# sovrasov/3d-object-detection.pytorch

Hardware: AMD Instinct MI355X
Metric: regression train crops/sec @224^2 bs256 MobileNetV2 (higher is better)
Workload: dtype bf16; 1 GPU; mobilenetv2 9-class Objectron keypoint regression, train step (fwd + l1/add/CE losses + bwd + AdamW), 224x224 crops, per-GPU batch 256; global_batch=256, parallelism=dp1, roofline_sampled_steps=0, rccl_ranks=0

## Files before the change

### 3d-object-detection.pytorch_amd/csrc/bn.hip

```cpp
#include "common.h"

namespace {

__device__ __forceinline__ void load_sums(const double* __restrict__ stats, int nrep, long long rstride, int C, int c, int rl,
                                          double& s1, double& s2) {
  s1 = 0.0;
  s2 = 0.0;
  if (c < C) {
    for (int r = rl; r < nrep; r += 16) {
      s1 += stats[r * rstride + c];
      s2 += stats[r * rstride + C + c];
    }
  }
#pragma unroll
  for (int o = 8; o > 0; o >>= 1) {
    s1 += __shfl_xor(s1, o, 16);
    s2 += __shfl_xor(s2, o, 16);
  }
}

__global__ void bn_finalize_kernel(const double* __restrict__ stats, int nrep, long long rstride, int C, double count,
                                   const float* __restrict__ gamma, const float* __restrict__ beta,
                                   float* running_mean, float* running_var, int64_t* nbt, float momentum,
                                   float eps, float* scale, float* shift, float* mean_out, float* invstd_out) {
// ... 50 lines not shown
__global__ void bn_bwd_finalize_kernel(const double* __restrict__ stats, int nrep, long long rstride, int C, double count,
                                       const float* __restrict__ gamma, const float* __restrict__ mean,
                                       const float* __restrict__ invstd, float* alpha, float* beta, float* gammac,
                                       float* dgamma, float* dbeta) {
  const int c = blockIdx.x * 16 + (threadIdx.x >> 4), rl = threadIdx.x & 15;
  double s1, s2;
  load_sums(stats, nrep, rstride, C, c, rl, s1, s2);
  if (c >= C || rl != 0) return;
  const double mu = (double)mean[c], is = (double)invstd[c];
  const double dg = is * (s2 - mu * s1);
  const double a = (double)(gamma ? gamma[c] : 1.f) * is;
  const double b = -a * is * dg / count;
  alpha[c] = (float)a;
  beta[c] = (float)b;
  gammac[c] = (float)(-a * s1 / count - b * mu);
  if (dgamma) dgamma[c] = (float)dg;
  if (dbeta) dbeta[c] = (float)s1;
}

__global__ __launch_bounds__(256) void bn_fold_kernel(const T3dFold* __restrict__ fp) {
  __shared__ float sink[3 * 64];
  const int C = fp->C, cbase = blockIdx.x * 64;
  if (cbase >= C) return;
  t3d_fold_block(fp, cbase, min(64, C - cbase), sink, 64, true);
}

}

int t3d_fold_fallback(const void* key, hipStream_t st) {
  const T3dFold* d = t3d_take_fold(key);
  if (!d) return T3D_OK;
  T3D_LAUNCH(bn_fold_kernel, dim3(32), dim3(256), 0, st, d);
  T3D_CHECK_LAUNCH();
  return T3D_OK;
}

extern "C" int t3d_bn_finalize(const double* stats, int C, double count, const float* gamma, const float* beta,
                               float* running_mean, float* running_var, int64_t* num_batches_tracked,
                               float momentum, float eps, float* scale, float* shift, float* mean, float* invstd,
                               void* stream) {
  if (!stats || !scale || !shift || C <= 0 || count <= 0) return T3D_ERR_ARG;
  T3D_LAUNCH(bn_finalize_kernel, dim3(cdiv(C, 16)), dim3(256), 0, reinterpret_cast<hipStream_t>(stream),
                     stats, g_t3d_reduce.nrep, g_t3d_reduce.stats_stride, C, count, gamma, beta, running_mean, running_var, num_batches_tracked, momentum, eps,
                     scale, shift, mean, invstd);
  T3D_CHECK_LAUNCH();
  return T3D_OK;
}
// ... 31 lines not shown
```

### 3d-object-detection.pytorch_amd/csrc/common.h

```cpp
#pragma once
#include <hip/hip_runtime.h>
#include <hip/hip_ext.h>
#include <stdint.h>
#include <type_traits>
#include "../../include/t3d.h"

typedef __bf16 bf16_t;
typedef __attribute__((ext_vector_type(8))) __bf16 bf16x8;
typedef __attribute__((ext_vector_type(4))) __bf16 bf16x4;
typedef _Float16 f16_t;
typedef __attribute__((ext_vector_type(8))) _Float16 f16x8;
typedef __attribute__((ext_vector_type(4))) float f32x4;
typedef __attribute__((ext_vector_type(2))) float f32x2;
__device__ __forceinline__ f32x2 pk_fma(f32x2 a, f32x2 b, f32x2 c) { return __builtin_elementwise_fma(a, b, c); }

#define T3D_CHECK_LAUNCH()                                  \
  do {                                                      \
    hipError_t e_ = hipGetLastError();                      \
    if (e_ != hipSuccess) return T3D_ERR_LAUNCH;            \
  } while (0)

static inline int cdiv(int a, int b) { return (a + b - 1) / b; }

hipError_t t3d_max_lds(const void* fn, int bytes);
// ... 34 lines not shown
                                           \
      if (g_t3d_signal.ev && g_t3d_signal.stream == (st)) (void)hipEventRecord(g_t3d_signal.ev, st);                     \
    } else {                                                                                                             \
      T3D_LAUNCH(kernel, grid, block, lds, st, __VA_ARGS__);                                                             \
    }                                                                                                                    \
  } while (0)

struct T3dWorkspace { void* ptr; long long bytes; };
extern T3dWorkspace g_t3d_ws;
extern T3dWorkspace g_t3d_ws_main;

typedef t3d_bn_fold T3dFold;
struct T3dFoldReq { const T3dFold* desc; const void* key; };
extern T3dFoldReq g_t3d_fold;
inline const T3dFold* t3d_take_fold(const void* key) {
  if (!key || !g_t3d_fold.desc || g_t3d_fold.key != key) return nullptr;
  const T3dFold* d = g_t3d_fold.desc;
  g_t3d_fold.desc = nullptr;
  return d;
}

int t3d_fold_fallback(const void* key, hipStream_t st);

struct T3dNoop { __device__ __forceinline__ void operator()() const {} };
template <class Between = T3dNoop>
__device__ __forceinline__ void t3d_fold_block(const T3dFold* __restrict__ fp, int cbase, int Cb, float* dst, int ld,
                                               bool publish, Between between = Between()) {
  const T3dFold f = *fp;
  const int nthr = blockDim.x;
  auto finish = [&](int i, double s1, double s2) {
    const int c = cbase + i;
    if (f.kind == 1) {
      const double mean = s1 / f.count;
      double var = s2 / f.count - mean * mean;
      if (var < 0.0) var = 0.0;
      const float invstd = (float)(1.0 / sqrt(var + (double)f.eps));
      const float g = f.gamma ? f.gamma[c] : 1.f, b = f.beta ? f.beta[c] : 0.f;
      const float sc = g * invstd, sh = b - (float)mean * sc;
      dst[i] = sc;
      dst[ld + i] = sh;
      if (publish) {
        f.o0[c] = sc;
        f.o1[c] = sh;
        if (f.o2) f.o2[c] = (float)mean;
        if (f.o3) f.o3[c] = invstd;
        if (f.rm) f.rm[c] = (1.f - f.momentum) * f.rm[c] + f.momentum * (float)mean;
        if (f.rv) {
          const double unbiased = f.count > 1.0 ? var * f.count / (f.count - 1.0) : var;
          f.rv[c] = (1.f - f.momentum) * f.rv[c] + f.momentum * (float)unbiased;
        }
        if (c == 0 && f.nbt) *f.nbt += 1;
      }
    } else {
      const double mu = (double)f.mean[c], is = (double)f.invstd[c];
      const double dg = is * (s2 - mu * s1);
      const double al = (double)(f.gamma ? f.gamma[c] : 1.f) * is;
      const double be = -al * is * dg / f.count;
      const float ga = (float)(-al * s1 / f.count - be * mu);
      dst[i] = (float)al;
      dst[ld + i] = (float)be;
      dst[2 * ld + i] = ga;
      if (publish) {
        f.o0[c] = (float)al;
        f.o1[c] = (float)be;
        f.o2[c] = ga;
        if (f.o3) f.o3[c] = (float)dg;
        if (f.o4) f.o4[c] = (float)s1;
      }
    }
  };
  auto pass = [&](auto nr_tag, auto u_tag) {
    constexpr int NR = decltype(nr_tag)::value, U = decltype(u_tag)::value;
    bool first = true;
    for (int i0 = threadIdx.x; i0 < Cb || first; i0 += U * nthr) {
      double v1[U][NR], v2[U][NR];
#pragma unroll
      for (int u = 0; u < U; ++u) {
        const int i = min(i0 + u * nthr, Cb - 1);
        const double* p = f.stats + cbase + i;
#pragma unroll
        for (int r = 0; r < NR; ++r) {
          const size_t o = (size_t)min(r, f.nrep - 1) * f.rstride;
          v1[u][r] = p[o];
          v2[u][r] = p[o + f.C];
        }
      }
      if (first) {
        between();
        first = false;
      }
#pragma unroll
      for (int u = 0; u < U; ++u) {
        double s1 = 0.0, s2 = 0.0;
#pragma unroll
        for (int r = 0; r < NR; ++r) {
          s1 += r < f.nrep ? v1[u][r] : 0.0;
          s2 += r < f.nrep ? v2[u][r] : 0.0;
        }
        if (i0 + u * nthr < Cb) finish(i0 + u * nthr, s1, s2);
      }
    }
  };
  if (f.nrep <= 2) pass(std::integral_constant<int, 2>{}, std::integral_constant<int, 8>{});
  else if (f.nrep <= 4) pass(std::integral_constant<int, 4>{}, std::integral_constant<int, 4>{});
  else if (f.nrep <= 8) pass(std::integral_constant<int, 8>{}, std::integral_constant<int, 2>{});
  else pass(std::integral_constant<int, 16>{}, std::integral_constant<int, 1>{});
  __syncthreads();
}

struct T3dQuant { double q, iq; };
static inline T3dQuant t3d_quant_for(long long count) {
  int e = 0;
  while ((1LL << e) < count) ++e;
  const double q = ldexp(1.0, e - 40);
  return T3dQuant{q, 1.0 / q};
}
__device__ __forceinline__ double t3d_snap(float v, const T3dQuant& t, bool squares) {
  if (t.q == 0.0) return (double)v;
  const double s = squares ? 1024.0 : 1.0;
  return rint((double)v * (t.iq * (1.0 / s))) * (t.q * s);
}

template <typename T> struct Vec8;
template <> struct Vec8<float> {
  static __device__ __forceinline__ void load(const float* p, float v[8]) {
    const float4 a = *reinterpret_cast<const float4*>(p);
    const float4 b = *reinterpret_cast<const float4*>(p + 4);
    v[0] = a.x; v[1] = a.y; v[2] = a.z; v[3] = a.w; v[4] = b.x; v[5] = b.y; v[6] = b.z; v[7] = b.w;
  }
  static __device__ __forceinline__ void store(float* p, const float v[8]) {
// ... 154 lines not shown
```

### 3d-object-detection.pytorch_amd/csrc/dwconv3_bwd_stream.hip

```cpp
#include <cstdlib>
#include <type_traits>
#include "dwconv_route.h"

namespace {

struct Dw3BArgs {
  const void *dz, *y, *x, *res;
  void* dx;
  const float* w;
  const float *alpha, *beta, *gamma;
  int per_sample;
  const float *scale, *shift;
  int act;
  double* stats;
  float* dw;
  int B, H, W, C;
  int rows_per_chunk, nchunks, slab, nitems;
  int nrep;
  long long rstride;
  int dw_slots;
  int* dw_used;
  int noflush;
  const T3dFold* fold;
};
// ... 53 lines not shown
    qstride = gridDim.y;
  } else {
    cg = blockIdx.y * 64 + (threadIdx.x & 63);
    on = cg < CG;
    if (!on) cg = 0;
    q0 = blockIdx.x * (NTH / 64) + __builtin_amdgcn_readfirstlane(threadIdx.x >> 6);
    qstride = gridDim.x * (NTH / 64);
  }
  const int c0 = cg * CH;
  const bool affine = a.scale != nullptr || ACT != T3D_ACT_NONE;
  const int cbase = a.slab ? blockIdx.y * 64 * CH : 0;
  const int Cb = a.slab ? min(64 * CH, a.C - cbase) : a.C;
  f32x2 wreg[9];
  const float* wl = lred + (c0 - cbase);
  if constexpr (CH == 2) {
#pragma unroll
    for (int t = 0; t < 9; ++t) wreg[t] = f32x2{a.w[(size_t)c0 * 9 + t], a.w[(size_t)(c0 + 1) * 9 + t]};
  } else {
    for (int i = threadIdx.x; i < 9 * Cb; i += NTH) lred[i] = a.w[(size_t)(cbase + i % Cb) * 9 + i / Cb];
    __syncthreads();
  }

  float* fco = lred + 9 * Cb;
  if (a.fold) t3d_fold_block(a.fold, cbase, Cb, fco, Cb, a.slab ? blockIdx.x == 0 : (blockIdx.x == 0 && blockIdx.y == 0));
  f32x2 sc2[H2], sh2[H2], al2[H2], be2[H2], ga2[H2];
  f32x2 wacc[9][H2];
  float psum[CH], psq[CH];
#pragma unroll
  for (int h = 0; h < H2; ++h) {
    const int c = c0 + 2 * h;
    sc2[h] = f32x2{a.scale ? a.scale[c] : 1.f, a.scale ? a.scale[c + 1] : 1.f};
    sh2[h] = f32x2{a.scale ? a.shift[c] : 0.f, a.scale ? a.shift[c + 1] : 0.f};
    if (a.fold) {
      const float* fc = fco + (c - cbase);
      al2[h] = f32x2{fc[0], fc[1]};
      be2[h] = f32x2{fc[Cb], fc[Cb + 1]};
      ga2[h] = f32x2{fc[2 * Cb], fc[2 * Cb + 1]};
    } else {
      be2[h] = f32x2{a.beta[c], a.beta[c + 1]};
      al2[h] = a.per_sample ? f32x2{0.f, 0.f} : f32x2{a.alpha[c], a.alpha[c + 1]};
      ga2[h] = a.per_sample ? f32x2{0.f, 0.f} : f32x2{a.gamma[c], a.gamma[c + 1]};
    }
#pragma unroll
    for (int t = 0; t < 9; ++t) wacc[t][h] = f32x2{0.f, 0.f};
  }
#pragma unroll
  for (int i = 0; i < CH; ++i) psum[i] = psq[i] = 0.f;
// ... 386 lines not shown
  extern __shared__ float lred[];
  using RV = rawvec<T, CH>;
  const int CG = a.C / CH, Ho = (a.H - 1) / 2 + 1, Wo = (a.W - 1) / 2 + 1;
  int cg, ow_fixed = 0, q0, qstride;
  bool on;
  if (!a.slab) {
    const int j = blockIdx.x * NTH + threadIdx.x;
    on = j < Wo * CG;
    cg = on ? j % CG : 0;
    ow_fixed = on ? j / CG : 0;
    q0 = blockIdx.y;
    qstride = gridDim.y;
  } else {
    cg = blockIdx.y * 64 + (threadIdx.x & 63);
    on = cg < CG;
    if (!on) cg = 0;
    q0 = blockIdx.x * (NTH / 64) + __builtin_amdgcn_readfirstlane(threadIdx.x >> 6);
    qstride = gridDim.x * (NTH / 64);
  }
  const int c0 = cg * CH;
  const bool affine = a.scale != nullptr || act_rt != T3D_ACT_NONE;
  const int cbase = a.slab ? blockIdx.y * 64 * CH : 0;
  const int Cb = a.slab ? min(64 * CH, a.C - cbase) : a.C;
  if (a.fold) t3d_fold_block(a.fold, cbase, Cb, lred, Cb, a.slab ? blockIdx.x == 0 : (blockIdx.x == 0 && blockIdx.y == 0));

  f32x2 sc2[H2], sh2[H2], al2[H2], be2[H2], ga2[H2];
  f32x2 wt[9][H2], wacc[9][H2];
  float psum[CH], psq[CH];
  {
    float wb[CH * 9];
    const float4* wp = reinterpret_cast<const float4*>(a.w + (size_t)c0 * 9);
#pragma unroll
    for (int i = 0; i < CH * 9 / 4; ++i) {
      const float4 q = wp[i];
      wb[4 * i] = q.x; wb[4 * i + 1] = q.y; wb[4 * i + 2] = q.z; wb[4 * i + 3] = q.w;
    }
#pragma unroll
    for (int h = 0; h < H2; ++h) {
      const int c = c0 + 2 * h;
      sc2[h] = f32x2{a.scale ? a.scale[c] : 1.f, a.scale ? a.scale[c + 1] : 1.f};
      sh2[h] = f32x2{a.scale ? a.shift[c] : 0.f, a.scale ? a.shift[c + 1] : 0.f};
      if (a.fold) {
        const float* fc = lred + (c - cbase);
        al2[h] = f32x2{fc[0], fc[1]};
        be2[h] = f32x2{fc[Cb], fc[Cb + 1]};
        ga2[h] = f32x2{fc[2 * Cb], fc[2 * Cb + 1]};
      } else {
// ... 310 lines not shown
```

### 3d-object-detection.pytorch_amd/csrc/dwconv3_stream.hip

```cpp
#include <cstdlib>
#include "dwconv_route.h"

namespace {

struct Dw3Args {
  const void* x;
  void* y;
  const float* w;
  const float *scale, *shift;
  int act;
  double* stats;
  int B, H, W, C, Ho, Wo;
  int rows_per_chunk, nchunks;
  int slab;
  int nitems;
  T3dQuant quant;
  int nrep;
  long long rstride;
  const T3dFold* fold;
};

template <typename T, int CH> using rawvec = T __attribute__((ext_vector_type(CH)));

template <typename RV>
// ... 58 lines not shown
  constexpr int H2 = CH / 2;
  extern __shared__ __attribute__((aligned(16))) float lstat[];
  using RV = rawvec<T, CH>;
  const int CG = a.C / CH;
  int cg, ox_fixed = 0, q0, qstride;
  bool on;
  if (!a.slab) {
    const int j = blockIdx.x * 256 + threadIdx.x;
    on = j < a.Wo * CG;
    cg = on ? j % CG : 0;
    ox_fixed = on ? j / CG : 0;
    q0 = blockIdx.y;
    qstride = gridDim.y;
  } else {
    cg = blockIdx.y * 64 + (threadIdx.x & 63);
    on = cg < CG;
    if (!on) cg = 0;
    q0 = blockIdx.x * 4 + __builtin_amdgcn_readfirstlane(threadIdx.x >> 6);
    qstride = gridDim.x * 4;
  }
  const int c0 = cg * CH;
  const bool affine = a.scale != nullptr || ACT != T3D_ACT_NONE;
  const int fbase = a.slab ? blockIdx.y * 64 * CH : 0, fCb = a.slab ? min(64 * CH, a.C - fbase) : a.C;
  if (a.fold) t3d_fold_block(a.fold, fbase, fCb, lstat, fCb, a.slab ? blockIdx.x == 0 : (blockIdx.x == 0 && blockIdx.y == 0));

  float wt[9][CH], sc[CH], sh[CH], psum[CH], psq[CH];
  {
    float wb[CH * 9];
    const float4* wp = reinterpret_cast<const float4*>(a.w + (size_t)c0 * 9);
#pragma unroll
    for (int i = 0; i < CH * 9 / 4; ++i) {
      const float4 q = wp[i];
      wb[4 * i] = q.x; wb[4 * i + 1] = q.y; wb[4 * i + 2] = q.z; wb[4 * i + 3] = q.w;
    }
#pragma unroll
    for (int i = 0; i < CH; ++i) {
      sc[i] = a.fold ? lstat[c0 - fbase + i] : (a.scale ? a.scale[c0 + i] : 1.f);
      sh[i] = a.fold ? lstat[fCb + c0 - fbase + i] : (a.scale ? a.shift[c0 + i] : 0.f);
      psum[i] = psq[i] = 0.f;
#pragma unroll
      for (int t = 0; t < 9; ++t) wt[t][i] = wb[i * 9 + t] * (C6 ? 6.f : 1.f);
      if (C6) { sc[i] *= T3D_SIXTH; sh[i] *= T3D_SIXTH; }
    }
  }
  f32x2 sc2[H2], sh2[H2];
#pragma unroll
  for (int h = 0; h < H2; ++h) { sc2[h] = f32x2{sc[2 * h], sc[2 * h + 1]}; sh2[h] = f32x2{sh[2 * h], sh[2 * h + 1]}; }
// ... 190 lines not shown
    qstride = gridDim.y;
  } else {
    cg = blockIdx.y * 64 + (threadIdx.x & 63);
    on = cg < CG;
    if (!on) cg = 0;
    q0 = blockIdx.x * 4 + __builtin_amdgcn_readfirstlane(threadIdx.x >> 6);
    qstride = gridDim.x * 4;
  }
  const int c0 = cg * CH;
  const bool affine = a.scale != nullptr || ACT != T3D_ACT_NONE;
  const int fbase = a.slab ? blockIdx.y * 64 * CH : 0, fCb = a.slab ? min(64 * CH, a.C - fbase) : a.C;
  f32x2 w2[9][H2], sc2[H2], sh2[H2];
  f32x2 psum[H2], psq[H2];
  {
    float wb[CH * 9];
    auto load_w = [&]() {
      const float4* wp = reinterpret_cast<const float4*>(a.w + (size_t)c0 * 9);
#pragma unroll
      for (int i = 0; i < CH * 9 / 4; ++i) {
        const float4 q = wp[i];
        wb[4 * i] = q.x; wb[4 * i + 1] = q.y; wb[4 * i + 2] = q.z; wb[4 * i + 3] = q.w;
      }
    };
    if (a.fold) t3d_fold_block(a.fold, fbase, fCb, lstat, fCb, a.slab ? blockIdx.x == 0 : (blockIdx.x == 0 && blockIdx.y == 0), load_w);
    else load_w();
#pragma unroll
    for (int h = 0; h < H2; ++h) {
      if (a.fold) {
        sc2[h] = f32x2{lstat[c0 - fbase + 2 * h], lstat[c0 - fbase + 2 * h + 1]};
        sh2[h] = f32x2{lstat[fCb + c0 - fbase + 2 * h], lstat[fCb + c0 - fbase + 2 * h + 1]};
      } else {
        sc2[h] = f32x2{a.scale ? a.scale[c0 + 2 * h] : 1.f, a.scale ? a.scale[c0 + 2 * h + 1] : 1.f};
        sh2[h] = f32x2{a.scale ? a.shift[c0 + 2 * h] : 0.f, a.scale ? a.shift[c0 + 2 * h + 1] : 0.f};
      }
#pragma unroll
      for (int t = 0; t < 9; ++t) w2[t][h] = f32x2{wb[(2 * h) * 9 + t], wb[(2 * h + 1) * 9 + t]};
      if (C6) {
        sc2[h] = sc2[h] * f32x2{T3D_SIXTH, T3D_SIXTH};
        sh2[h] = sh2[h] * f32x2{T3D_SIXTH, T3D_SIXTH};
#pragma unroll
        for (int t = 0; t < 9; ++t) w2[t][h] = w2[t][h] * f32x2{6.f, 6.f};
      }
      psum[h] = psq[h] = f32x2{0.f, 0.f};
    }
  }
  if (a.fold) __syncthreads();

// ... 243 lines not shown
```

### 3d-object-detection.pytorch_amd/csrc/elementwise.hip

```cpp
#include "common.h"

namespace {

template <typename T, bool U8>
__global__ __launch_bounds__(256) void im2col_kernel(const void* __restrict__ xin, const float* __restrict__ mean,
                                                     const float* __restrict__ istd, T* __restrict__ col, int B,
                                                     int H, int W, int Ho, int Wo) {
  extern __shared__ float tile[];
  const int WP = W + 2;
  const int hp = (Ho + 1) / 2;
  const int b = blockIdx.x / hp, oy0 = (blockIdx.x % hp) * 2;
  const int iy0 = oy0 * 2 - 1;
  const int tid = threadIdx.x;
  for (int i = tid; i < 15 * 2; i += 256) {
    const int rr = i >> 1;
    tile[rr * WP + ((i & 1) ? W + 1 : 0)] = 0.f;
  }
  if constexpr (U8) {
    const unsigned char* xu = reinterpret_cast<const unsigned char*>(xin);
    const float mu[3] = {mean[0], mean[1], mean[2]}, is[3] = {istd[0], istd[1], istd[2]};
    const int RB = W * 3;
    if ((RB & 3) == 0) {
      const int R4 = RB >> 2;
      for (int i = tid; i < 5 * R4; i += 256) {
// ... 83 lines not shown
  for (int i = threadIdx.x; i < 2 * C; i += blockDim.x) lstat[i] = 0.0;
  __syncthreads();
  if (on) {
#pragma unroll
    for (int i = 0; i < 8; ++i) {
      atomicAdd(lstat + c0 + i, (double)s1[i]);
      atomicAdd(lstat + C + c0 + i, (double)s2[i]);
    }
  }
  __syncthreads();
  for (int i = threadIdx.x; i < 2 * C; i += blockDim.x) atomicAdd(stats + i, lstat[i]);
}

template <typename T>
__global__ __launch_bounds__(256) void bn_apply_kernel(const EwArgs a) {
  const int CG = a.C / 8;
  const size_t nvec = (size_t)a.M * CG;
  const T* __restrict__ y = reinterpret_cast<const T*>(a.a);
  const T* __restrict__ r = reinterpret_cast<const T*>(a.res);
  T* __restrict__ z = reinterpret_cast<T*>(a.out);
  const size_t nthr = ((size_t)gridDim.x * 256 / CG) * CG;
  const size_t g = blockIdx.x * (size_t)256 + threadIdx.x;
  extern __shared__ float fco[];
  if (a.fold) t3d_fold_block(a.fold, 0, a.C, fco, a.C, blockIdx.x == 0);
  if (g >= nthr) return;
  const int c0 = (int)(g % CG) * 8;
  float sc[8], sh[8];
  if (a.fold) {
#pragma unroll
    for (int i = 0; i < 8; ++i) { sc[i] = fco[c0 + i]; sh[i] = fco[a.C + c0 + i]; }
  } else {
    load_affine(a, c0, sc, sh);
  }
  for (size_t i = g; i < nvec; i += nthr) {
    float v[8];
    Vec8<T>::load(y + i * 8, v);
    act_affine_vec<8>(v, sc, sh, a.act);
    if (r) {
      float rr[8];
      Vec8<T>::load(r + i * 8, rr);
#pragma unroll
      for (int j = 0; j < 8; ++j) v[j] += rr[j];
    }
    Vec8<T>::store(z + i * 8, v);
  }
}

// ... 402 lines not shown
```

### 3d-object-detection.pytorch_amd/csrc/misc.hip

```cpp
#include "common.h"

namespace {

template <typename T>
__global__ void pack_kernel(const float* __restrict__ w, T* __restrict__ out, int rows, int cols, int transpose) {
  const size_t n = (size_t)rows * cols;
  for (size_t i = blockIdx.x * (size_t)blockDim.x + threadIdx.x; i < n; i += (size_t)gridDim.x * blockDim.x) {
    if (!transpose) {
      out[i] = (T)w[i];
    } else {
      const size_t r = i / cols, c = i % cols;
      out[c * rows + r] = (T)w[i];
    }
  }
}

__device__ __forceinline__ size_t t3d_frag_piece(int r, int c8, int KS) {
  const int rr = r & 31, T = (r >> 5) * 2 + ((rr >> 2) & 1), lc = (rr >> 3) * 4 + (rr & 3);
  return ((size_t)T * KS + (c8 >> 2)) * 64 + (c8 & 3) * 16 + lc;
}

template <typename T>
__global__ void pack_batched_kernel(const long long* __restrict__ desc) {
  const long long* d = desc + (size_t)blockIdx.x * 7;
// ... 226 lines not shown
  for (int r = 0; r < nrep; ++r) {
    sy += fstats[r * rstride + c];
    sdz += bstats[r * rstride + c];
  }
  dbias[c] = (float)((double)alpha[c] * sdz + (double)beta[c] * sy + count * (double)gammac[c]);
}

__global__ void se_bwd_affine_kernel(const float* __restrict__ s, const float* __restrict__ g,
                                     const float* __restrict__ alpha, const float* __restrict__ gammac,
                                     float* __restrict__ aps, float* __restrict__ gps, int B, int C) {
  const int n = B * C;
  for (int i = blockIdx.x * blockDim.x + threadIdx.x; i < n; i += gridDim.x * blockDim.x) {
    const int c = i % C;
    aps[i] = s[i] * alpha[c];
    gps[i] = gammac[c] + g[i] * alpha[c];
  }
}

__global__ __launch_bounds__(256) void se_bwd_affine_fold_kernel(const float* __restrict__ s, const float* __restrict__ g,
                                                                 const T3dFold* __restrict__ fold, float* __restrict__ aps,
                                                                 float* __restrict__ gps, int B, int C) {
  __shared__ float co[3][32];
  const int c0 = blockIdx.x * 32, cb = min(32, C - c0);
  t3d_fold_block(fold, c0, cb, &co[0][0], 32, blockIdx.y == 0);
  const int per = (B + gridDim.y - 1) / gridDim.y, b0 = blockIdx.y * per, b1 = min(B, b0 + per);
  for (int i = b0 * 32 + threadIdx.x; i < b1 * 32; i += 256) {
    const int b = i >> 5, cl = i & 31;
    if (cl < cb) {
      const size_t o = (size_t)b * C + c0 + cl;
      aps[o] = s[o] * co[0][cl];
      gps[o] = co[2][cl] + g[o] * co[0][cl];
    }
  }
}

__device__ __forceinline__ void philox_round(uint32_t c[4], uint32_t k0, uint32_t k1) {
  const uint64_t p0 = (uint64_t)0xD2511F53u * c[0], p1 = (uint64_t)0xCD9E8D57u * c[2];
  const uint32_t n0 = (uint32_t)(p1 >> 32) ^ c[1] ^ k0, n2 = (uint32_t)(p0 >> 32) ^ c[3] ^ k1;
  c[1] = (uint32_t)p1; c[3] = (uint32_t)p0; c[0] = n0; c[2] = n2;
}
__global__ void dropout_mask_kernel(float* __restrict__ mask, long long n, unsigned long long seed,
                                    unsigned long long offset, float keep, float scale) {
  const long long n4 = (n + 3) / 4;
  for (long long i = blockIdx.x * (long long)blockDim.x + threadIdx.x; i < n4; i += (long long)gridDim.x * blockDim.x) {
    uint32_t c[4] = {(uint32_t)i, (uint32_t)(i >> 32), (uint32_t)offset, (uint32_t)(offset >> 32)};
    uint32_t k0 = (uint32_t)seed, k1 = (uint32_t)(seed >> 32);
#pragma unroll
// ... 260 lines not shown
```

### 3d-object-detection.pytorch_amd/csrc/pwconv_deep.hip

```cpp
#include <cstdlib>
#include <type_traits>
#include "pwconv_route.h"

namespace t3d_pw {
namespace {

__device__ __forceinline__ f32x2 deep_fma_clamp01(f32x2 a, f32x2 b, f32x2 c) {
  f32x2 d;
  asm("v_pk_fma_f32 %0, %1, %2, %3 clamp" : "=v"(d) : "v"(a), "v"(b), "v"(c));
  return d;
}

#ifdef T3D_PW_TRACE
__device__ unsigned long long g_deep_trace[16];
#define DEEP_STAMP(i)                                                                                     \
  do {                                                                                                    \
    if (threadIdx.x == 0 && blockIdx.y == 0 && (blockIdx.x == 0 || blockIdx.x == gridDim.x - 1))         \
      g_deep_trace[(blockIdx.x == 0 ? 0 : 8) + (i)] = wall_clock64();                                     \
  } while (0)
#else
#define DEEP_STAMP(i)
#endif

constexpr int RT = 4;
// ... 51 lines not shown
    constexpr int SL = decltype(slot_tag)::value;
#pragma unroll
    for (int j = 0; j < IT; ++j) {
      const size_t o = arow + min((ph * KSP + sks + j) * 32, a.Kin - 8 - lg * 8);
      pa[SL][j] = *reinterpret_cast<const bf16x8*>(A0 + o);
      if (DG) pb[DG ? SL : 0][DG ? j : 0] = *reinterpret_cast<const bf16x8*>(A1 + o);
    }
  };
  w_issue(std::integral_constant<int, 0>{}, 0);
  a_issue(std::integral_constant<int, 0>{}, 0);
  a_issue(std::integral_constant<int, 1>{}, 1);

  for (int i = tid; i < BN * 2; i += 64 * NW) dstat[i] = 0.0;
  for (int i = tid; i < BN; i += 64 * NW) {
    const int n = n0 + i;
    const bool v = DG && a.e_scale && n < a.Nout;
    ecoef[i] = v ? a.e_scale[n] : 1.f;
    ecoef[BN + i] = v ? a.e_shift[n] : 0.f;
  }
  if (a.fold) {
    for (int i = a.Kin + tid; i < kpad; i += 64 * NW) {
      coef[i] = DG ? 0.f : 1.f; coef[kpad + i] = 0.f; coef[2 * kpad + i] = 0.f;
    }
    t3d_fold_block(a.fold, 0, a.Kin, coef, kpad, blockIdx.x == 0 && blockIdx.y == 0);
  } else {
    for (int i = tid; i < kpad; i += 64 * NW) {
      const bool v = i < a.Kin;
      if (!DG) {
        coef[i] = (v && a.p0) ? a.p0[i] : 1.f;
        coef[kpad + i] = (v && a.p0) ? a.p1[i] : 0.f;
      } else {
        coef[i] = v ? a.p0[i] : 0.f;
        coef[kpad + i] = v ? a.p1[i] : 0.f;
        coef[2 * kpad + i] = v ? a.p2[i] : 0.f;
      }
    }
    __syncthreads();
  }
  const bool c6f = !DG && a.p0 && a.act == T3D_ACT_RELU6;
  if (c6f) {
    for (int i = tid; i < 2 * kpad; i += 64 * NW) coef[i] *= T3D_SIXTH;
    __syncthreads();
  }
  const int fact = c6f ? -1 : a.act;
  DEEP_STAMP(1);

  f32x4 acc[RT][NTW];
// ... 238 lines not shown
```

### 3d-object-detection.pytorch_amd/csrc/pwconv_stream.hip

```cpp
#include <cstdlib>
#include <type_traits>
#include "pwconv_route.h"

#ifndef T3D_PW_F16
typedef bf16_t ST;
typedef bf16x8 ST8;
#define T3D_PW_MFMA __builtin_amdgcn_mfma_f32_16x16x32_bf16
#define T3D_PW_LAUNCH stream_launch
#define T3D_PW_CAN stream_can
#else
typedef f16_t ST;
typedef f16x8 ST8;
#define T3D_PW_MFMA __builtin_amdgcn_mfma_f32_16x16x32_f16
#define T3D_PW_LAUNCH stream_launch_f16
#define T3D_PW_CAN stream_f16_can
#endif

namespace t3d_pw {
__device__ __forceinline__ f32x2 pk_fma_clamp01(f32x2 a, f32x2 b, f32x2 c) {
  f32x2 d;
  asm("v_pk_fma_f32 %0, %1, %2, %3 clamp" : "=v"(d) : "v"(a), "v"(b), "v"(c));
  return d;
}

namespace {


#ifdef T3D_PW_TRACE
__device__ unsigned long long g_pw_trace[16];
#define PW_STAMP(i)                                                                                       \
  do {                                                                                                    \
    if (threadIdx.x == 0 && (blockIdx.x == 0 || blockIdx.x == gridDim.x - 1))                            \
      g_pw_trace[(blockIdx.x == 0 ? 0 : 8) + (i)] = wall_clock64();                                       \
  } while (0)
#else
#define PW_STAMP(i)
#endif

template <int NT, int R, bool DG, bool GEN, bool YF = false, int KU = 2, bool ZM = false>
__global__ __launch_bounds__(512, KU > 2 ? 1 : 2) void pw_stream_kernel(const GemmArgs a, const int nchunks, const int KS, const int nrep, const long long rstride) {
  constexpr int BN = NT * 16;
  extern __shared__ __attribute__((aligned(16))) unsigned char smem[];
  ST8* Wf = reinterpret_cast<ST8*>(smem);
  const int kpad = KS * 32;
  float* coef = reinterpret_cast<float*>(smem + (size_t)NT * KS * 1024);
  float* lstat = coef + 3 * kpad;
  float* ecoef = lstat + BN * 2;
  double* dstat = reinterpret_cast<double*>(ecoef + 2 * BN);

  const int tid = threadIdx.x, lane = tid & 63, wave = tid >> 6;
  const int lg = lane >> 4, lc = lane & 15;
  const int nxb = gridDim.x / nchunks;
  int chunk, xb;
// ... 52 lines not shown
#pragma unroll
      for (int u = 0; u < SU; ++u) {
        if (!ok[u]) {
#pragma unroll
          for (int j = 0; j < 8; ++j) v[u][j] = (ST)0.f;
        }
        if (i0 + u * nthr < total) Wf[i0 + u * nthr] = v[u];
      }
    }
  }
  for (int i = tid; i < BN * 2; i += nthr) { lstat[i] = 0.f; dstat[i] = 0.0; }
  for (int i = tid; i < BN; i += nthr) {
    const int n = n0 + i;
    const bool v = DG && a.e_scale && n < a.Nout;
    ecoef[i] = v ? a.e_scale[n] : 1.f;
    ecoef[BN + i] = v ? a.e_shift[n] : 0.f;
  }
  };
  constexpr bool DGL = DG && !YF;
  if (!YF && a.fold) {
    for (int i = a.Kin + tid; i < kpad; i += nthr) {
      coef[i] = DG ? 0.f : 1.f; coef[kpad + i] = 0.f; coef[2 * kpad + i] = 0.f;
    }
    t3d_fold_block(a.fold, 0, a.Kin, coef, kpad, blockIdx.x == 0, stage_weights);
  } else {
  stage_weights();
  for (int i = tid; i < kpad; i += nthr) {
    const bool v = i < a.Kin;
    if (YF) {
      coef[i] = 1.f; coef[kpad + i] = 0.f; coef[2 * kpad + i] = 0.f;
    } else if (!DG) {
      coef[i] = (v && a.p0) ? a.p0[i] : 1.f;
      coef[kpad + i] = (v && a.p0) ? a.p1[i] : 0.f;
    } else {
      coef[i] = (v && !a.per_sample) ? a.p0[i] : 0.f;
      coef[kpad + i] = v ? a.p1[i] : 0.f;
      coef[2 * kpad + i] = (v && !a.per_sample) ? a.p2[i] : 0.f;
    }
  }
  }
  __syncthreads();
  const bool c6f = !DG && !ZM && !YF && a.act == T3D_ACT_RELU6 && !(GEN && a.p2);
  if (c6f) {
    for (int i = tid; i < 2 * kpad; i += nthr) coef[i] *= T3D_SIXTH;
    __syncthreads();
  }
  PW_STAMP(1);
// ... 306 lines not shown
        const float s1 = row16_sum(st1[q][j]), s2 = row16_sum(st2[q][j]);
        st1[q][j] = st2[q][j] = 0.f;
        if (lc == 0 && n < a.Nout && g_begin < g_end) {
          atomicAdd(dstat + (n - n0 + j) * 2, (double)s1);
          atomicAdd(dstat + (n - n0 + j) * 2 + 1, (double)s2);
        }
      }
    }
    __syncthreads();
    for (int i = tid; i < BN * 2; i += nthr) {
      const int n = n0 + (i >> 1);
      if (n < a.Nout) a.ps_stats[((size_t)sb * a.Nout + n) * 2 + (i & 1)] = (float)dstat[i];
      dstat[i] = 0.0;
    }
    __syncthreads();
  }
  }
  PW_STAMP(3);

  if (keep_stats) {
#pragma unroll
    for (int q = 0; q < NT / 2; ++q) {
      const int n = nb + 32 * q;
#pragma unroll
      for (int j = 0; j < 8; ++j) {
        const float s1 = row16_sum(st1[q][j]), s2 = row16_sum(st2[q][j]);
        if (lc == 0 && n < a.Nout) {
          atomicAdd(dstat + (n - n0 + j) * 2, t3d_snap(s1, a.quant, false));
          atomicAdd(dstat + (n - n0 + j) * 2 + 1, t3d_snap(s2, a.quant, !DG));
        }
      }
    }
    __syncthreads();
    for (int i = tid; i < BN * 2; i += nthr) {
      const int n = n0 + (i >> 1);
      if (n < a.Nout) atomicAdd(a.stats + (size_t)(xb % nrep) * rstride + (size_t)(i & 1) * a.Nout + n, dstat[i]);
    }
  }
  PW_STAMP(4);
}

template <int NT, int R, bool DG, bool GEN, bool YF = false, int KU = 2, bool ZM = false>
int launch_v(GemmArgs& a, int KS, hipStream_t st) {
  constexpr int BN = NT * 16;
  const int kpad = KS * 32;
  const size_t lds = (size_t)NT * KS * 1024 + (size_t)3 * kpad * 4 + BN * 4 * 4 + BN * 2 * 8;
  const int nchunks = cdiv(a.Nout, BN);
  const int ngroups = cdiv(a.M, 16 * R);
  const bool ps = GEN && a.ps_stats != nullptr;
  const int gps = cdiv(a.HW, 16 * R);
  const int threads = (lds <= 48 * 1024 || (ps && gps <= 4)) ? 256 : 512;
  const void* fn = (const void*)pw_stream_kernel<NT, R, DG, GEN, YF, KU, ZM>;
  if (lds > 64 * 1024) (void)t3d_max_lds(fn, (int)lds);
// ... 93 lines not shown
```

### 3d-object-detection.pytorch_amd/csrc/pwconv_wgrad_tr.hip

```cpp
#include <cstdlib>
#include "pwconv_route.h"

namespace {

__device__ __forceinline__ f32x2 pk_fma_clamp01(f32x2 a, f32x2 b, f32x2 c) {
  f32x2 d;
  asm("v_pk_fma_f32 %0, %1, %2, %3 clamp" : "=v"(d) : "v"(a), "v"(b), "v"(c));
  return d;
}

typedef __attribute__((ext_vector_type(4))) short s16x4;

__device__ __forceinline__ void act_vec8(float* v, int act) {
  switch (act) {
    case T3D_ACT_RELU:
#pragma unroll
      for (int j = 0; j < 8; ++j) v[j] = fmaxf(v[j], 0.f);
      break;
    case T3D_ACT_RELU6:
#pragma unroll
      for (int j = 0; j < 8; ++j) v[j] = __builtin_amdgcn_fmed3f(v[j], 0.f, 6.f);
      break;
    case T3D_ACT_HSWISH:
#pragma unroll
// ... 61 lines not shown
  int tile, split;
  {
    const int L = blockIdx.x;
    if (ntiles > 1 && L < ntiles * s8) {
      const int j = L >> 3;
      tile = j % ntiles;
      split = (j / ntiles) * 8 + (L & 7);
    } else {
      const int Lr = ntiles > 1 ? L - ntiles * s8 : L;
      tile = Lr % ntiles;
      split = (ntiles > 1 ? s8 : 0) + Lr / ntiles;
    }
  }
  const int pt = tile / a.qtiles, qt = tile % a.qtiles;
  const int p0 = pt * PB, q0 = qt * QB;
  const int mbeg = split * a.rows_per_split, mend = min(a.M, mbeg + a.rows_per_split);
  constexpr int dyB = SWAP ? QB : PB, aB = SWAP ? PB : QB;
  const int dy0 = SWAP ? q0 : p0, a0c = SWAP ? p0 : q0;
  float* cdy = coef;
  float* ca = coef + 3 * dyB;
  if (!YF && a.fold) {
    const int nv = min(dyB, a.N - dy0);
    for (int i = nv + threadIdx.x; i < dyB; i += 256 * G) cdy[i] = cdy[dyB + i] = cdy[2 * dyB + i] = 0.f;
    t3d_fold_block(a.fold, dy0, nv, cdy, dyB, false);
  } else {
  for (int i = threadIdx.x; i < dyB && !YF; i += 256 * G) {
    const int n = dy0 + i;
    const bool v = n < a.N;
    cdy[i] = (v && !a.per_sample) ? a.alpha[n] : 0.f;
    cdy[dyB + i] = v ? a.beta[n] : 0.f;
    cdy[2 * dyB + i] = (v && !a.per_sample) ? a.gamma[n] : 0.f;
  }
  }
  const bool c6 = !GEN && !YF && a.act == T3D_ACT_RELU6 && !a.se;
  for (int i = threadIdx.x; i < aB; i += 256 * G) {
    const int k = a0c + i;
    const bool v = k < a.K;
    ca[i] = ((v && a.scale) ? a.scale[k] : 1.f) * (c6 ? T3D_SIXTH : 1.f);
    ca[aB + i] = ((v && a.scale) ? a.shift[k] : 0.f) * (c6 ? T3D_SIXTH : 1.f);
  }
  float* const gsl = coef + ((NCOEF + 3) & ~3);
  const int gs_b0 = GEN ? mbeg / a.HW : 0;
  if constexpr (GEN == 2) {
    {
      const int nb = a.M / a.HW;
      for (int i = threadIdx.x; i < a.gs_ns * aB; i += 256 * G) {
        const int sb = i / aB, c = i % aB, b = min(gs_b0 + sb, nb - 1), k = a0c + c;
        gsl[i] = k < a.K ? a.se[(size_t)b * a.K + k] : 0.f;
      }
    }
  }
  if constexpr (DGF) {
    if (a.wd) {
      for (int i = threadIdx.x; i < QB * (PB / 8); i += 256 * G) {
        const int r = i / (PB / 8), c = (i % (PB / 8)) * 8;
        *reinterpret_cast<bf16x8*>(wdl + r * RSW + c) = *reinterpret_cast<const bf16x8*>(a.wd + (size_t)r * PB + c);
      }
    } else {
      const int Nz = a.Nz, K = a.K;
      float* fco = cdy;
      if (a.fold) {
        for (int i = Nz + threadIdx.x; i < dyB; i += 256 * G) fco[i] = fco[dyB + i] = fco[2 * dyB + i] = 0.f;
        t3d_fold_block(a.fold, 0, Nz, fco, dyB, blockIdx.x == 0);
      } else {
        for (int i = threadIdx.x; i < dyB; i += 256 * G) {
          const bool v = i < Nz;
          fco[i] = v ? a.alpha[i] : 0.f; fco[dyB + i] = v ? a.beta[i] : 0.f; fco[2 * dyB + i] = v ? a.gamma[i] : 0.f;
        }
      }
      for (int i = threadIdx.x; i < QB * (RSW / 8); i += 256 * G) *reinterpret_cast<bf16x8*>(wdl + i * 8) = bf16x8{};
      __syncthreads();
      const float *alpha = fco, *beta = fco + dyB, *gamma = fco + 2 * dyB;
      const bf16_t* __restrict__ wtr = a.wtr;
      for (int i = threadIdx.x; i < QB * (Nz / 8); i += 256 * G) {
        const int k = i / (Nz / 8), n = (i % (Nz / 8)) * 8;
        if (k < K) {
          const bf16x8 v = *reinterpret_cast<const bf16x8*>(wtr + (size_t)k * Nz + n);
          bf16x8 o;
#pragma unroll
          for (int j = 0; j < 8; ++j) o[j] = (bf16_t)(alpha[n + j] * (float)v[j]);
          *reinterpret_cast<bf16x8*>(wdl + k * RSW + n) = o;
        }
      }
      f32x4* qred = reinterpret_cast<f32x4*>(tiles);
      const int lgq_ = lane >> 4, lcq_ = lane & 15;
      const int nst = (Nz + 31) / 32;
// ... 667 lines not shown
```

### 3d-object-detection.pytorch_amd/csrc/pwconv_yfree.hip

```cpp
#include "pwconv_route.h"

int t3d_pw_wgrad_tr_yfree(const void* dz, const void* x, float* tmp, int M, int HW, int K, int N, hipStream_t st);
size_t t3d_pw_bwd_yfree_scratch(int M, int K, int N);
int t3d_pw_bwd_yfree_launch(const void* dz, const void* x, const void* wd, const void* wt, const t3d_bnbwd* bb, const void* x_raw,
                            const void* residual, void* dx, double* stats, void* scratch, int M, int HW, int K, int N, hipStream_t st);
int t3d_pw_bwd_yfree_reduce(void* scratch, float** tmp_out, int M, int K, int N, hipStream_t st);

namespace {

__global__ __launch_bounds__(256) void yfree_prep_kernel(const bf16_t* __restrict__ wt, const float* __restrict__ alpha_g,
                                                         const float* __restrict__ beta_g, const float* __restrict__ gamma_g,
                                                         bf16_t* __restrict__ wcat, float* __restrict__ cvec, int K, int N,
                                                         int NP, int KP, const T3dFold* __restrict__ fold,
                                                         bf16_t* __restrict__ wd, int PBw) {
  extern __shared__ float fco[];
  __shared__ f32x4 red[3][64];
  const int t = threadIdx.x, lane = t & 63, wave = t >> 6, lg = lane >> 4, lc = lane & 15;
  if (fold) {
    t3d_fold_block(fold, 0, N, fco, N, blockIdx.x == 0 && blockIdx.y == 0);
  } else {
    for (int i = t; i < N; i += 256) { fco[i] = alpha_g[i]; fco[N + i] = beta_g[i]; fco[2 * N + i] = gamma_g[i]; }
    __syncthreads();
  }
  const float *alpha = fco, *beta = fco + N, *gamma = fco + 2 * N;
  const int tot = NP + KP;
  const int k0 = blockIdx.x * 16, q0 = blockIdx.y * 16;
  f32x4 acc = {0.f, 0.f, 0.f, 0.f};
  const int nsteps = (N + 31) / 32;
  const int ka = min(k0 + lc, K - 1), kb = min(q0 + lc, K - 1);
  const bf16_t* ra = wt + (size_t)ka * N;
  const bf16_t* rb = wt + (size_t)kb * N;
  constexpr int U = 4;
  for (int s0 = wave; s0 < nsteps; s0 += 4 * U) {
    bf16x8 fa[U], fb[U];
#pragma unroll
    for (int u = 0; u < U; ++u) {
      const int n = min((s0 + 4 * u) * 32 + 8 * lg, N - 8);
      fa[u] = *reinterpret_cast<const bf16x8*>(ra + n);
      fb[u] = *reinterpret_cast<const bf16x8*>(rb + n);
    }
#pragma unroll
    for (int u = 0; u < U; ++u) {
// ... 186 lines not shown
```

Before: 38340 crops/s.

## Specialize BN fold block by kind at compile time and skip idle waves

The BN-fold helper that runs in the prologue of many fused kernels now takes the fold kind as a template parameter, so each call site compiles only the forward or backward path and loads just the fields it needs. It no longer copies the whole descriptor struct, and it gates the stats loads per wave so waves with no channels to process skip them. The aim is lower register pressure and prologue latency in the host kernels. Separately, the pwconv stats epilogue spreads its per-channel atomics across lanes instead of serializing 16 atomics on a single lane, and optional trace stamps are added. The nrep<=2 specialization is dropped, so those cases now fall into the 4-wide path.

```diff
diff --git a/3d-object-detection.pytorch_amd/csrc/bn.hip b/3d-object-detection.pytorch_amd/csrc/bn.hip
--- a/3d-object-detection.pytorch_amd/csrc/bn.hip
+++ b/3d-object-detection.pytorch_amd/csrc/bn.hip
@@ -96,7 +96,7 @@
   __shared__ float sink[3 * 64];
   const int C = fp->C, cbase = blockIdx.x * 64;
   if (cbase >= C) return;
-  t3d_fold_block(fp, cbase, min(64, C - cbase), sink, 64, true);
+  t3d_fold_block<0>(fp, cbase, min(64, C - cbase), sink, 64, true);
 }
 
 }
diff --git a/3d-object-detection.pytorch_amd/csrc/common.h b/3d-object-detection.pytorch_amd/csrc/common.h
--- a/3d-object-detection.pytorch_amd/csrc/common.h
+++ b/3d-object-detection.pytorch_amd/csrc/common.h
@@ -80,90 +80,129 @@
 
 int t3d_fold_fallback(const void* key, hipStream_t st);
 
+#ifndef T3D_FOLD_STAMP
+#define T3D_FOLD_STAMP(i)
+#endif
 struct T3dNoop { __device__ __forceinline__ void operator()() const {} };
-template <class Between = T3dNoop>
+template <int KIND, class Between = T3dNoop>
 __device__ __forceinline__ void t3d_fold_block(const T3dFold* __restrict__ fp, int cbase, int Cb, float* dst, int ld,
                                                bool publish, Between between = Between()) {
-  const T3dFold f = *fp;
-  const int nthr = blockDim.x;
-  auto finish = [&](int i, double s1, double s2) {
-    const int c = cbase + i;
-    if (f.kind == 1) {
-      const double mean = s1 / f.count;
-      double var = s2 / f.count - mean * mean;
-      if (var < 0.0) var = 0.0;
-      const float invstd = (float)(1.0 / sqrt(var + (double)f.eps));
-      const float g = f.gamma ? f.gamma[c] : 1.f, b = f.beta ? f.beta[c] : 0.f;
-      const float sc = g * invstd, sh = b - (float)mean * sc;
-      dst[i] = sc;
-      dst[ld + i] = sh;
-      if (publish) {
-        f.o0[c] = sc;
-        f.o1[c] = sh;
-        if (f.o2) f.o2[c] = (float)mean;
-        if (f.o3) f.o3[c] = invstd;
-        if (f.rm) f.rm[c] = (1.f - f.momentum) * f.rm[c] + f.momentum * (float)mean;
-        if (f.rv) {
-          const double unbiased = f.count > 1.0 ? var * f.count / (f.count - 1.0) : var;
-          f.rv[c] = (1.f - f.momentum) * f.rv[c] + f.momentum * (float)unbiased;
-        }
-        if (c == 0 && f.nbt) *f.nbt += 1;
+  if constexpr (KIND == 0) {
+    if (fp->kind == 1) t3d_fold_block<1>(fp, cbase, Cb, dst, ld, publish, between);
+    else t3d_fold_block<2>(fp, cbase, Cb, dst, ld, publish, between);
+  } else {
+    const int nthr = blockDim.x, lane = threadIdx.x & 63;
+    const int wbase = __builtin_amdgcn_readfirstlane((int)threadIdx.x - lane);
+    const bool live = wbase < Cb;
+    int nrep = 16, C = 0;
+    long long rstride = 0;
+    const double* stats = nullptr;
+    double count = 1.0;
+    float eps = 0.f;
+    const float *pa = nullptr, *pb = nullptr, *pc = nullptr;
+    if (live) {
+      nrep = fp->nrep; C = fp->C; rstride = fp->rstride; stats = fp->stats; count = fp->count;
+      if (KIND == 1) { eps = fp->eps; pa = fp->gamma; pb = fp->beta; }
+      else { pa = fp->mean; pb = fp->invstd; pc = fp->gamma; }
+    }
+    T3D_FOLD_STAMP(0);
+    auto finish = [&](int i, double s1, double s2, float xa, float xb, float xc) {
+      const int c = cbase + i;
+      if (KIND == 1) {
+        const double mean = s1 / count;
+        double var = s2 / count - mean * mean;
+        if (var < 0.0) var = 0.0;
+        const float invstd = (float)(1.0 / sqrt(var + (double)eps));
+        const float g = xa, b = xb;
+        const float sc = g * invstd, sh = b - (float)mean * sc;
+        dst[i] = sc;
+        dst[ld + i] = sh;
+        if (publish) {
+          float* const o2 = fp->o2; float* const o3 = fp->o3; float* const rm = fp->rm; float* const rv = fp->rv;
+          const float momentum = fp->momentum;
+          fp->o0[c] = sc;
+          fp->o1[c] = sh;
+          if (o2) o2[c] = (float)mean;
+          if (o3) o3[c] = invstd;
+          if (rm) rm[c] = (1.f - momentum) * rm[c] + momentum * (float)mean;
+          if (rv) {
+            const double unbiased = count > 1.0 ? var * count / (count - 1.0) : var;
+            rv[c] = (1.f - momentum) * rv[c] + momentum * (float)unbiased;
+          }
+          if (c == 0 && fp->nbt) *fp->nbt += 1;
+        }
+      } else {
+        const double mu = (double)xa, is = (double)xb;
+        const double dg = is * (s2 - mu * s1);
+        const double al = (double)xc * is;
+        const double be = -al * is * dg / count;
+        const float ga = (float)(-al * s1 / count - be * mu);
+        dst[i] = (float)al;
+        dst[ld + i] = (float)be;
+        dst[2 * ld + i] = ga;
+        if (publish) {
+          float* const o3 = fp->o3; float* const o4 = fp->o4;
+          fp->o0[c] = (float)al;
+          fp->o1[c] = (float)be;
+          fp->o2[c] = ga;
+          if (o3) o3[c] = (float)dg;
+          if (o4) o4[c] = (float)s1;
+        }
       }
-    } else {
-      const double mu = (double)f.mean[c], is = (double)f.invstd[c];
-      const double dg = is * (s2 - mu * s1);
-      const double al = (double)(f.gamma ? f.gamma[c] : 1.f) * is;
-      const double be = -al * is * dg / f.count;
-      const float ga = (float)(-al * s1 / f.count - be * mu);
-      dst[i] = (float)al;
-      dst[ld + i] = (float)be;
-      dst[2 * ld + i] = ga;
-      if (publish) {
-        f.o0[c] = (float)al;
-        f.o1[c] = (float)be;
-        f.o2[c] = ga;
-        if (f.o3) f.o3[c] = (float)dg;
-        if (f.o4) f.o4[c] = (float)s1;
+    };
+    auto pass = [&](auto nr_tag, auto u_tag) {
+      constexpr int NR = decltype(nr_tag)::value, U = decltype(u_tag)::value;
+      bool first = true;
+      for (int w0 = wbase; w0 < Cb || first; w0 += U * nthr) {
+        const int i0 = w0 + lane;
+        double v1[U][NR], v2[U][NR];
+        float xa[U], xb[U], xc[U];
+        if (w0 < Cb) {
+#pragma unroll
+          for (int u = 0; u < U; ++u) {
+            const int i = min(i0 + u * nthr, Cb - 1);
+            const double* p = stats + cbase + i;
+#pragma unroll
+            for (int r = 0; r < NR; ++r) {
+              const size_t o = (size_t)min(r, nrep - 1) * rstride;
+              v1[u][r] = p[o];
+              v2[u][r] = p[o + C];
+            }
+            if (KIND == 1) {
+              xa[u] = pa ? pa[cbase + i] : 1.f;
+              xb[u] = pb ? pb[cbase + i] : 0.f;
+              xc[u] = 0.f;
+            } else {
+              xa[u] = pa[cbase + i];
+              xb[u] = pb[cbase + i];
+              xc[u] = pc ? pc[cbase + i] : 1.f;
+            }
+          }
+        }
+        if (first) {
+          between();
+          first = false;
+          T3D_FOLD_STAMP(1);
+        }
+#pragma unroll
+        for (int u = 0; u < U; ++u) {
+          if (w0 + u * nthr >= Cb) continue;
+          double s1 = 0.0, s2 = 0.0;
+#pragma unroll
+          for (int r = 0; r < NR; ++r) {
+            s1 += r < nrep ? v1[u][r] : 0.0;
+            s2 += r < nrep ? v2[u][r] : 0.0;
+          }
+          if (i0 + u * nthr < Cb) finish(i0 + u * nthr, s1, s2, xa[u], xb[u], xc[u]);
+        }
       }
-    }
-  };
-  auto pass = [&](auto nr_tag, auto u_tag) {
-    constexpr int NR = decltype(nr_tag)::value, U = decltype(u_tag)::value;
-    bool first = true;
-    for (int i0 = threadIdx.x; i0 < Cb || first; i0 += U * nthr) {
-      double v1[U][NR], v2[U][NR];
-#pragma unroll
-      for (int u = 0; u < U; ++u) {
-        const int i = min(i0 + u * nthr, Cb - 1);
-        const double* p = f.stats + cbase + i;
-#pragma unroll
-        for (int r = 0; r < NR; ++r) {
-          const size_t o = (size_t)min(r, f.nrep - 1) * f.rstride;
-          v1[u][r] = p[o];
-          v2[u][r] = p[o + f.C];
-        }
-      }
-      if (first) {
-        between();
-        first = false;
-      }
-#pragma unroll
-      for (int u = 0; u < U; ++u) {
-        double s1 = 0.0, s2 = 0.0;
-#pragma unroll
-        for (int r = 0; r < NR; ++r) {
-          s1 += r < f.nrep ? v1[u][r] : 0.0;
-          s2 += r < f.nrep ? v2[u][r] : 0.0;
-        }
-        if (i0 + u * nthr < Cb) finish(i0 + u * nthr, s1, s2);
-      }
-    }
-  };
-  if (f.nrep <= 2) pass(std::integral_constant<int, 2>{}, std::integral_constant<int, 8>{});
-  else if (f.nrep <= 4) pass(std::integral_constant<int, 4>{}, std::integral_constant<int, 4>{});
-  else if (f.nrep <= 8) pass(std::integral_constant<int, 8>{}, std::integral_constant<int, 2>{});
-  else pass(std::integral_constant<int, 16>{}, std::integral_constant<int, 1>{});
-  __syncthreads();
+    };
+    if (nrep <= 4) pass(std::integral_constant<int, 4>{}, std::integral_constant<int, 4>{});
+    else if (nrep <= 8) pass(std::integral_constant<int, 8>{}, std::integral_constant<int, 2>{});
+    else pass(std::integral_constant<int, 16>{}, std::integral_constant<int, 1>{});
+    T3D_FOLD_STAMP(2);
+    __syncthreads();
+  }
 }
 
 struct T3dQuant { double q, iq; };
diff --git a/3d-object-detection.pytorch_amd/csrc/dwconv3_bwd_stream.hip b/3d-object-detection.pytorch_amd/csrc/dwconv3_bwd_stream.hip
--- a/3d-object-detection.pytorch_amd/csrc/dwconv3_bwd_stream.hip
+++ b/3d-object-detection.pytorch_amd/csrc/dwconv3_bwd_stream.hip
@@ -99,7 +99,7 @@
   }
 
   float* fco = lred + 9 * Cb;
-  if (a.fold) t3d_fold_block(a.fold, cbase, Cb, fco, Cb, a.slab ? blockIdx.x == 0 : (blockIdx.x == 0 && blockIdx.y == 0));
+  if (a.fold) t3d_fold_block<2>(a.fold, cbase, Cb, fco, Cb, a.slab ? blockIdx.x == 0 : (blockIdx.x == 0 && blockIdx.y == 0));
   f32x2 sc2[H2], sh2[H2], al2[H2], be2[H2], ga2[H2];
   f32x2 wacc[9][H2];
   float psum[CH], psq[CH];
@@ -532,7 +532,7 @@
   const bool affine = a.scale != nullptr || act_rt != T3D_ACT_NONE;
   const int cbase = a.slab ? blockIdx.y * 64 * CH : 0;
   const int Cb = a.slab ? min(64 * CH, a.C - cbase) : a.C;
-  if (a.fold) t3d_fold_block(a.fold, cbase, Cb, lred, Cb, a.slab ? blockIdx.x == 0 : (blockIdx.x == 0 && blockIdx.y == 0));
+  if (a.fold) t3d_fold_block<2>(a.fold, cbase, Cb, lred, Cb, a.slab ? blockIdx.x == 0 : (blockIdx.x == 0 && blockIdx.y == 0));
 
   f32x2 sc2[H2], sh2[H2], al2[H2], be2[H2], ga2[H2];
   f32x2 wt[9][H2], wacc[9][H2];
diff --git a/3d-object-detection.pytorch_amd/csrc/dwconv3_stream.hip b/3d-object-detection.pytorch_amd/csrc/dwconv3_stream.hip
--- a/3d-object-detection.pytorch_amd/csrc/dwconv3_stream.hip
+++ b/3d-object-detection.pytorch_amd/csrc/dwconv3_stream.hip
@@ -104,7 +104,7 @@
   const int c0 = cg * CH;
   const bool affine = a.scale != nullptr || ACT != T3D_ACT_NONE;
   const int fbase = a.slab ? blockIdx.y * 64 * CH : 0, fCb = a.slab ? min(64 * CH, a.C - fbase) : a.C;
-  if (a.fold) t3d_fold_block(a.fold, fbase, fCb, lstat, fCb, a.slab ? blockIdx.x == 0 : (blockIdx.x == 0 && blockIdx.y == 0));
+  if (a.fold) t3d_fold_block<1>(a.fold, fbase, fCb, lstat, fCb, a.slab ? blockIdx.x == 0 : (blockIdx.x == 0 && blockIdx.y == 0));
 
   float wt[9][CH], sc[CH], sh[CH], psum[CH], psq[CH];
   {
@@ -341,7 +341,7 @@
         wb[4 * i] = q.x; wb[4 * i + 1] = q.y; wb[4 * i + 2] = q.z; wb[4 * i + 3] = q.w;
       }
     };
-    if (a.fold) t3d_fold_block(a.fold, fbase, fCb, lstat, fCb, a.slab ? blockIdx.x == 0 : (blockIdx.x == 0 && blockIdx.y == 0), load_w);
+    if (a.fold) t3d_fold_block<1>(a.fold, fbase, fCb, lstat, fCb, a.slab ? blockIdx.x == 0 : (blockIdx.x == 0 && blockIdx.y == 0), load_w);
     else load_w();
 #pragma unroll
     for (int h = 0; h < H2; ++h) {
diff --git a/3d-object-detection.pytorch_amd/csrc/elementwise.hip b/3d-object-detection.pytorch_amd/csrc/elementwise.hip
--- a/3d-object-detection.pytorch_amd/csrc/elementwise.hip
+++ b/3d-object-detection.pytorch_amd/csrc/elementwise.hip
@@ -129,7 +129,7 @@
   const size_t nthr = ((size_t)gridDim.x * 256 / CG) * CG;
   const size_t g = blockIdx.x * (size_t)256 + threadIdx.x;
   extern __shared__ float fco[];
-  if (a.fold) t3d_fold_block(a.fold, 0, a.C, fco, a.C, blockIdx.x == 0);
+  if (a.fold) t3d_fold_block<1>(a.fold, 0, a.C, fco, a.C, blockIdx.x == 0);
   if (g >= nthr) return;
   const int c0 = (int)(g % CG) * 8;
   float sc[8], sh[8];
diff --git a/3d-object-detection.pytorch_amd/csrc/misc.hip b/3d-object-detection.pytorch_amd/csrc/misc.hip
--- a/3d-object-detection.pytorch_amd/csrc/misc.hip
+++ b/3d-object-detection.pytorch_amd/csrc/misc.hip
@@ -272,7 +272,7 @@
                                                                  float* __restrict__ gps, int B, int C) {
   __shared__ float co[3][32];
   const int c0 = blockIdx.x * 32, cb = min(32, C - c0);
-  t3d_fold_block(fold, c0, cb, &co[0][0], 32, blockIdx.y == 0);
+  t3d_fold_block<2>(fold, c0, cb, &co[0][0], 32, blockIdx.y == 0);
   const int per = (B + gridDim.y - 1) / gridDim.y, b0 = blockIdx.y * per, b1 = min(B, b0 + per);
   for (int i = b0 * 32 + threadIdx.x; i < b1 * 32; i += 256) {
     const int b = i >> 5, cl = i & 31;
diff --git a/3d-object-detection.pytorch_amd/csrc/pwconv_deep.hip b/3d-object-detection.pytorch_amd/csrc/pwconv_deep.hip
--- a/3d-object-detection.pytorch_amd/csrc/pwconv_deep.hip
+++ b/3d-object-detection.pytorch_amd/csrc/pwconv_deep.hip
@@ -97,7 +97,7 @@
     for (int i = a.Kin + tid; i < kpad; i += 64 * NW) {
       coef[i] = DG ? 0.f : 1.f; coef[kpad + i] = 0.f; coef[2 * kpad + i] = 0.f;
     }
-    t3d_fold_block(a.fold, 0, a.Kin, coef, kpad, blockIdx.x == 0 && blockIdx.y == 0);
+    t3d_fold_block<DG ? 2 : 1>(a.fold, 0, a.Kin, coef, kpad, blockIdx.x == 0 && blockIdx.y == 0);
   } else {
     for (int i = tid; i < kpad; i += 64 * NW) {
       const bool v = i < a.Kin;
diff --git a/3d-object-detection.pytorch_amd/csrc/pwconv_stream.hip b/3d-object-detection.pytorch_amd/csrc/pwconv_stream.hip
--- a/3d-object-detection.pytorch_amd/csrc/pwconv_stream.hip
+++ b/3d-object-detection.pytorch_amd/csrc/pwconv_stream.hip
@@ -1,5 +1,15 @@
 #include <cstdlib>
 #include <type_traits>
+#ifdef T3D_PW_TRACE
+#include <hip/hip_runtime.h>
+static __device__ unsigned long long g_pw_trace[16];
+#define T3D_FOLD_STAMP(i)                                                                                 \
+  do {                                                                                                    \
+    asm volatile("s_waitcnt vmcnt(0) lgkmcnt(0)" ::: "memory");                                           \
+    if (threadIdx.x == 0 && (blockIdx.x == 0 || blockIdx.x == gridDim.x - 1))                            \
+      g_pw_trace[(blockIdx.x == 0 ? 0 : 8) + 5 + (i)] = wall_clock64();                                   \
+  } while (0)
+#endif
 #include "pwconv_route.h"
 
 #ifndef T3D_PW_F16
@@ -27,8 +37,7 @@
 
 
 #ifdef T3D_PW_TRACE
-__device__ unsigned long long g_pw_trace[16];
-#define PW_STAMP(i)                                                                                       \
+#define PW_STAMP(i)                                                                                     \
   do {                                                                                                    \
     if (threadIdx.x == 0 && (blockIdx.x == 0 || blockIdx.x == gridDim.x - 1))                            \
       g_pw_trace[(blockIdx.x == 0 ? 0 : 8) + (i)] = wall_clock64();                                       \
@@ -127,7 +136,7 @@
     for (int i = a.Kin + tid; i < kpad; i += nthr) {
       coef[i] = DG ? 0.f : 1.f; coef[kpad + i] = 0.f; coef[2 * kpad + i] = 0.f;
     }
-    t3d_fold_block(a.fold, 0, a.Kin, coef, kpad, blockIdx.x == 0, stage_weights);
+    t3d_fold_block<DG ? 2 : 1>(a.fold, 0, a.Kin, coef, kpad, blockIdx.x == 0, stage_weights);
   } else {
   stage_weights();
   for (int i = tid; i < kpad; i += nthr) {
@@ -480,13 +489,15 @@
 #pragma unroll
     for (int q = 0; q < NT / 2; ++q) {
       const int n = nb + 32 * q;
+      float mine = 0.f;
 #pragma unroll
       for (int j = 0; j < 8; ++j) {
         const float s1 = row16_sum(st1[q][j]), s2 = row16_sum(st2[q][j]);
-        if (lc == 0 && n < a.Nout) {
-          atomicAdd(dstat + (n - n0 + j) * 2, t3d_snap(s1, a.quant, false));
-          atomicAdd(dstat + (n - n0 + j) * 2 + 1, t3d_snap(s2, a.quant, !DG));
-        }
+        mine = lc == j ? s1 : (lc == j + 8 ? s2 : mine);
+      }
+      if (n < a.Nout) {
+        const double d = lc < 8 ? t3d_snap(mine, a.quant, false) : t3d_snap(mine, a.quant, !DG);
+        atomicAdd(dstat + (n - n0 + (lc & 7)) * 2 + (lc >> 3), d);
       }
     }
     __syncthreads();
diff --git a/3d-object-detection.pytorch_amd/csrc/pwconv_wgrad_tr.hip b/3d-object-detection.pytorch_amd/csrc/pwconv_wgrad_tr.hip
--- a/3d-object-detection.pytorch_amd/csrc/pwconv_wgrad_tr.hip
+++ b/3d-object-detection.pytorch_amd/csrc/pwconv_wgrad_tr.hip
@@ -107,7 +107,7 @@
   if (!YF && a.fold) {
     const int nv = min(dyB, a.N - dy0);
     for (int i = nv + threadIdx.x; i < dyB; i += 256 * G) cdy[i] = cdy[dyB + i] = cdy[2 * dyB + i] = 0.f;
-    t3d_fold_block(a.fold, dy0, nv, cdy, dyB, false);
+    t3d_fold_block<2>(a.fold, dy0, nv, cdy, dyB, false);
   } else {
   for (int i = threadIdx.x; i < dyB && !YF; i += 256 * G) {
     const int n = dy0 + i;
@@ -146,7 +146,7 @@
       float* fco = cdy;
       if (a.fold) {
         for (int i = Nz + threadIdx.x; i < dyB; i += 256 * G) fco[i] = fco[dyB + i] = fco[2 * dyB + i] = 0.f;
-        t3d_fold_block(a.fold, 0, Nz, fco, dyB, blockIdx.x == 0);
+        t3d_fold_block<2>(a.fold, 0, Nz, fco, dyB, blockIdx.x == 0);
       } else {
         for (int i = threadIdx.x; i < dyB; i += 256 * G) {
           const bool v = i < Nz;
diff --git a/3d-object-detection.pytorch_amd/csrc/pwconv_yfree.hip b/3d-object-detection.pytorch_amd/csrc/pwconv_yfree.hip
--- a/3d-object-detection.pytorch_amd/csrc/pwconv_yfree.hip
+++ b/3d-object-detection.pytorch_amd/csrc/pwconv_yfree.hip
@@ -17,7 +17,7 @@
   __shared__ f32x4 red[3][64];
   const int t = threadIdx.x, lane = t & 63, wave = t >> 6, lg = lane >> 4, lc = lane & 15;
   if (fold) {
-    t3d_fold_block(fold, 0, N, fco, N, blockIdx.x == 0 && blockIdx.y == 0);
+    t3d_fold_block<2>(fold, 0, N, fco, N, blockIdx.x == 0 && blockIdx.y == 0);
   } else {
     for (int i = t; i < N; i += 256) { fco[i] = alpha_g[i]; fco[N + i] = beta_g[i]; fco[2 * N + i] = gamma_g[i]; }
     __syncthreads();
```

Result: faster. 38900 crops/s (median of 6 runs) (+1.5%).
